# sloisel/MultiGridBarrier.jl

Measured on NVIDIA B200. Metric: mgb_solve DOF*Newton-steps/s (fem2d_P1 ~1.6M DOF, p=1.5), higher is better.
Workload: dtype f64

## Files before the change

multigridbarrier.jl_b200/build.py:

```python
from __future__ import annotations

import os
import shutil
import subprocess
import sys
from concurrent.futures import ThreadPoolExecutor

HERE = os.path.dirname(os.path.abspath(__file__))
CSRC = os.path.join(HERE, "csrc")
OBJ = os.path.join(HERE, "build")
LIB = os.path.join(HERE, "libmgbx.so")
HDR = os.path.join("..", "..", "include", "mgbx.h")
ENGINE = ["engine.hpp", "host_sparse.hpp", "device_common.cuh", "elem_schur.cuh", "node_barrier.cuh", "pcg2.hpp", HDR]
SOURCES = {
    "mgbx.cu": ["mgbx.cu", "host_amg.hpp"] + ENGINE,
    "setup.cu": ["setup.cu", "setup_kernels.cuh"] + ENGINE,
    "evaluate.cu": ["evaluate.cu", "kernels.cuh", "dense_kernels.cuh"] + ENGINE,
    "linear_solve.cu": ["linear_solve.cu", "solver_kernels.cuh"] + ENGINE,
    "newton.cu": ["newton.cu"] + ENGINE,
    "pcg2.cu": ["pcg2.cu", "pcg2.hpp"],
}
FLAGS = ["-gencode", "arch=compute_100a,code=sm_100a", "-O3", "-DNDEBUG", "-lineinfo", "-std=c++17",
         "-Xcompiler", "-fPIC,-O2,-Wall,-Wno-unused-function"]


def nvcc_path():
    for c in (os.environ.get("NVCC"), shutil.which("nvcc"), "/usr/local/cuda/bin/nvcc"):
        if c and os.path.exists(c):
            return c
    raise RuntimeError("nvcc not found")


def _obj(src):
    return os.path.join(OBJ, os.path.splitext(src)[0] + ".o")


def _stale(src):
    o = _obj(src)
    if not os.path.exists(o):
        return True
    t = os.path.getmtime(o)
    return any(os.path.getmtime(os.path.join(CSRC, d)) > t for d in SOURCES[src])

# ... 37 lines not shown
```

multigridbarrier.jl_b200/csrc/device_common.cuh:

```cuda
#pragma once
#include <cuda_runtime.h>
#include <stdint.h>

#include "elem_schur.cuh"
#include "node_barrier.cuh"

namespace mgbx {

#define MGBX_MAX_OPS 8
constexpr int kRedBlocks = 592;
constexpr int kRedThreads = 256;

struct DevCsr {
  int64_t rows = 0, cols = 0, nnz = 0;
  int64_t *ptr = nullptr;
  int32_t *idx = nullptr;
  double *val = nullptr;
};

__device__ __forceinline__ double warp_sum(double v) {
#pragma unroll
  for (int o = 16; o > 0; o >>= 1) v += __shfl_down_sync(0xffffffffu, v, o);
  return v;
}
// ... 245 lines not shown
      "mbarrier.try_wait.parity.shared::cta.b64 p, [%0], %1;\n"
      "@p bra DONE_%=;\n"
      "bra WAIT_%=;\n"
      "DONE_%=:\n"
      "}\n" ::"r"(a),
      "r"(parity)
      : "memory");
}
__device__ __forceinline__ void bulk_g2s(void *smem, const void *gmem, unsigned int bytes, unsigned long long *bar) {
  asm volatile("cp.async.bulk.shared::cluster.global.mbarrier::complete_tx::bytes [%0], [%1], %2, [%3];" ::"r"((unsigned int)__cvta_generic_to_shared(smem)),
               "l"(gmem), "r"(bytes), "r"((unsigned int)__cvta_generic_to_shared(bar))
               : "memory");
}
__device__ __forceinline__ void fence_proxy_async_smem() { asm volatile("fence.proxy.async.shared::cta;" ::: "memory"); }

struct SellPlan {
  int64_t nout = 0, nslices = 0, nterms = 0;
  int64_t *sptr = nullptr;
  int32_t *cnt = nullptr;
  int32_t *src = nullptr;
  double *w = nullptr;
};

__device__ __forceinline__ int64_t csr_find(const DevCsr &A, int64_t row, int32_t col) {
  int64_t lo = A.ptr[row], hi = A.ptr[row + 1];
  while (lo < hi) {
    const int64_t mid = (lo + hi) >> 1;
    const int32_t c = A.idx[mid];
    if (c < col) lo = mid + 1;
    else if (c > col) hi = mid;
    else return mid;
  }
  return -1;
}

constexpr int kCoarseMaxDense = 128;
inline size_t coarse_inverse_smem(int m) { return sizeof(double) * ((size_t)m * (m + 1) + (size_t)m * (m + 1) / 2 + m); }
inline size_t dense_solve_small_smem(int m) { return sizeof(double) * ((size_t)m * (m + 1) + 2 * (size_t)m); }

constexpr int kGemmBM = 64, kGemmBN = 64, kGemmBK = 16, kGemmLd = kGemmBK + 4;

__device__ __forceinline__ void dmma_m8n8k4(double &d0, double &d1, double a, double b) {
  asm volatile("mma.sync.aligned.m8n8k4.row.col.f64.f64.f64.f64 {%0,%1}, {%2}, {%3}, {%0,%1};" : "+d"(d0), "+d"(d1) : "d"(a), "d"(b));
}

constexpr int kCholNB = 64;
// ... 28 lines not shown
```

multigridbarrier.jl_b200/csrc/engine.hpp:

```cpp
#pragma once
#include <cuda_runtime.h>

#include <chrono>
#include <cmath>
#include <cstdio>
#include <cstring>
#include <functional>
#include <map>
#include <memory>
#include <string>
#include <vector>

#include "host_sparse.hpp"
#include "device_common.cuh"
#include "pcg2.hpp"

namespace mgbx {

#define CK(call)                                                                                      \
  do {                                                                                                \
    cudaError_t e_ = (call);                                                                          \
    if (e_ != cudaSuccess)                                                                            \
      throw std::runtime_error(std::string("CUDA error: ") + cudaGetErrorString(e_) + " at " + __FILE__ + ":" + \
                               std::to_string(__LINE__));                                             \
// ... 210 lines not shown
constexpr int kScalPcgOut = 8;
constexpr int kScalTrialSeg = 38;
constexpr int kScalEvalDist = 40;
constexpr int kScalDotSeg = 44;
constexpr int kScalDotSeg2 = 50;
constexpr int kScalSlots = 64;
static_assert(kScalEval + 4 <= kScalDot && kScalDot + 3 <= kScalTrial && kScalTrial + 1 <= kScalSingle &&
                  kScalSingle <= kScalPcgOut && kScalPcgOut + kPcg2OutCount <= kScalTrialSeg &&
                  kScalTrialSeg + 2 == kScalEvalDist && kScalEvalDist + 4 == kScalDotSeg &&
                  kScalDotSeg + 6 <= kScalDotSeg2 && kScalDotSeg2 + 6 <= kScalSlots,
              "scalar slot regions overlap, break the all-reduced range or exceed dscal");

}

struct mgbx_handle {
  mgbx::Pool pool;
  mgbx::Amg amg[2];
  std::string err;
  mgbx_config cfg;
  cudaStream_t stream = nullptr;
  bool has_feas = false;
  double *partials = nullptr;
  unsigned int *ticket = nullptr;
  double *dscal = nullptr;
  double *hscal = nullptr;
  mgbx_step_result *res = nullptr;
  int64_t launches = 0;
  int64_t kc_launches[mgbx::KC_COUNT] = {0};
  double kc_ms[mgbx::KC_COUNT] = {0};
  std::vector<cudaEvent_t> ev_free;
  struct Pending {
    int kc;
    cudaEvent_t a, b;
  };
  std::vector<Pending> ev_pending;
  cudaEvent_t ev_cur = nullptr;
  int pcg2_grid = 0;
  double dgemm_flops = 0.0;
  mgbx::SolveTol last_tol{};
  int rank = 0, nranks = 1;
  void *comm = nullptr;
  int device = -1;
  std::vector<double> prof_ns;
  std::vector<int64_t> prof_cnt;
  std::vector<unsigned long long> prof_host;
};
// ... 73 lines not shown
  void copy(double *dst, const double *src, int64_t m) {
    if (m) CK(cudaMemcpyAsync(dst, src, sizeof(double) * m, cudaMemcpyDeviceToDevice, s));
  }
  void zero(double *dst, int64_t m) {
    if (m) CK(cudaMemsetAsync(dst, 0, sizeof(double) * m, s));
  }
  unsigned int red_grid(int64_t work) {
    const int64_t b = (work + kRedThreads - 1) / kRedThreads;
    return (unsigned int)std::max<int64_t>(1, std::min<int64_t>(b, kRedBlocks));
  }

  bool dist() const { return h->nranks > 1; }
  void allreduce(double *buf, int64_t count, int op = kNcclSum) {
    if (count > 0) NCK(nccl_api().AllReduce(buf, buf, (size_t)count, kNcclFloat64, op, h->comm, s));
  }
  SegList seglist(Amg &A, int J);
  void allreduce_shared(Amg &A, int J, double *v, double *extra = nullptr, int64_t nextra = 0);

  static int group_for(const DevCsr &A) {
    const double avg = A.rows ? (double)A.nnz / (double)A.rows : 0.0;
    return avg > 48.0 ? 32 : (avg > 6.0 ? 4 : 1);
  }
  void spmv(const DevCsr &A, const double *x, const double *y0, double alpha, double *y, int G = 0);
  void axpby(int64_t m, double a, const double *x, double b, const double *y, double *out);
  void prolong_to_fine(Amg &A, int J, const double *x, const double *zbase, double *zf);
  void restrict_from_fine(Amg &A, int J, const double *gb, double *gJ);
  Dot2 dot2(Amg &A, int J, const double *a, const double *b);
  MaxAbs maxabs(int64_t n, const double *v);
  TrialOut eval_trial(Amg &A, int J, double t, double sigma);
  void phase1_slack(Amg &A, Amg &F);
  void blockgrad(Amg &A, const ElemParams &E);
  NodeParams node_params(Amg &A, double t);
  ElemParams elem_params(Amg &A);
  bool elem_fused_setup(Amg &A, const NodeParams &NP, int nex, ElemFused &Q, size_t &smem, unsigned int &grid);
  int plap_dim(const Amg &A) const;
  bool plap_setup(Amg &A, int dim, double t, bool use_bw, PlapParams &Q, size_t &smem, unsigned int &grid, bool cond = true);
  EvalOut eval_f01(Amg &A, int J, double t, const double *zbase, const double *x, double *gout, bool use_bw = true,
                   double *step2 = nullptr);

  System &system_for(Amg &A, int J);
  void assemble(Amg &A, System &S, int J, double t, const double *zbase, const double *x);
  void assemble_unfused(Amg &A, System &S, int J, double t, const double *x);
  void galerkin(System &S, int kend);
  void schur_masks(const Amg &A, const System &S, unsigned &pieces, unsigned &elim) const;
  void assemble_dense(Amg &A, System &S, const NodeParams &P);
  void dgemm_nt(int M, int N, int K, const double *Am, int64_t lda, const double *Bm, int64_t ldb, const double *sc, double *C, int64_t ldc, bool acc, double alpha = 1.0);

  bool precond_fp32(const System &S) const;
  int lambda_power_its(const System &S) const;
  bool use_direct(const System &S, const SysLevel &Lv) const;
  std::vector<int> active_levels(const System &S, int ktop) const;
  void setup_hierarchy(Amg &A, System &S, int ktop);
  void dense_factor(SysLevel &Lv);
  void dense_apply(SysLevel &Lv, const double *b, double *x);
  void direct_solve(SysLevel &Lv, const double *b, double *x);
  SellBuild make_sell(const DevCsr &A, int64_t nthreads);
  void sell_prepare(System &S, int ktop);
  System::Pcg2Dev &pcg2_plan(System &S, int ktop);
  void pcg2_setup_dist(System::Pcg2Dev &D, int nshard);
  SolveResult pcg(System &S, int ktop, const double *b, double *x, const SolveTol &tol);
  SolveResult solve_compact(System &S, int ktop, const double *b, double *x, const SolveTol &tol);
  SolveResult solve(Amg &A, System &S, int J, const double *g, double *dir, const SolveTol &tol);

  struct NewtonOut {
    bool converged;
    int k;
    int status;
    double y, gnorm, inc;
  };
  NewtonOut newton(Amg &A, int J, double t, int maxit, int stop_kind, double lambda_tol, double theta, const mgbx_step_opts &o);
  int step(int which, double t, const mgbx_step_opts &o, mgbx_step_result *r);
  int matched_t(double t_default, double *t_out, double *tstar_out);
};

void solve_kernels_init();
void kron_w_init(size_t smem);

inline bool dense_mode(const Amg &A) { return A.N == 1 && A.p > 64; }

template <class F>
// ... 40 lines not shown
```

multigridbarrier.jl_b200/csrc/evaluate.cu:

```cuda
#include "engine.hpp"
#include "kernels.cuh"
#include "dense_kernels.cuh"

namespace mgbx {
namespace {

template <int MODE>
void launch_node(const NodeParams &P, unsigned int grid, cudaStream_t s) {
  if (P.nD <= 4) k_node<MODE, 4><<<grid, kRedThreads, 0, s>>>(P);
  else if (P.nD <= 6) k_node<MODE, 6><<<grid, kRedThreads, 0, s>>>(P);
  else if (P.nD <= 8) k_node<MODE, 8><<<grid, kRedThreads, 0, s>>>(P);
  else k_node<MODE, MGBX_MAX_ND><<<grid, kRedThreads, 0, s>>>(P);
}

template <auto K, class Params>
void launch_wave(const Params &Q, unsigned int grid, size_t smem, cudaStream_t s) {
  static int nsm[64] = {0};
  int dev = 0;
  CK(cudaGetDevice(&dev));
  if (!nsm[dev]) {
    CK(cudaFuncSetAttribute(K, cudaFuncAttributeMaxDynamicSharedMemorySize, 220 * 1024));
    CK(cudaDeviceGetAttribute(&nsm[dev], cudaDevAttrMultiProcessorCount, dev));
  }
  int occ = 1;
// ... 26 lines not shown
Dot2 dot2_slots(const double *d) { return {d[0], d[1], d[2]}; }
Dot2 dot2_seg_slots(const double *local, const double *shared) {
  return {local[0] + shared[0], local[1] + shared[1], local[2] + shared[2]};
}

}

void kron_w_init(size_t smem) { CK(cudaFuncSetAttribute(k_kron_w, cudaFuncAttributeMaxDynamicSharedMemorySize, (int)smem)); }

void Engine::spmv(const DevCsr &A, const double *x, const double *y0, double alpha, double *y, int G) {
  if (A.rows == 0) return;
  if (G == 0) G = group_for(A);
  pre_launch(KC_SPMV);
  if (G == 32) k_spmv<32><<<nblk(A.rows * 32), 256, 0, s>>>(A, x, y0, alpha, y);
  else if (G == 4) k_spmv<4><<<nblk(A.rows * 4), 256, 0, s>>>(A, x, y0, alpha, y);
  else k_spmv<1><<<nblk(A.rows), 256, 0, s>>>(A, x, y0, alpha, y);
  post_launch(KC_SPMV);
}

void Engine::axpby(int64_t m, double a, const double *x, double b, const double *y, double *out) {
  LAUNCH(KC_VEC, k_axpby<<<nblk(m), 256, 0, s>>>(m, a, x, b, y, out));
}

void Engine::prolong_to_fine(Amg &A, int J, const double *x, const double *zbase, double *zf) {
  const double *v = x;
  for (int l = J; l < A.L - 1; ++l) {
    spmv(A.T[l], v, nullptr, 1.0, A.chain[l + 1]);
    v = A.chain[l + 1];
  }
  spmv(A.RL, v, zbase, 1.0, zf);
}
void Engine::restrict_from_fine(Amg &A, int J, const double *gb, double *gJ) {
  if (J == A.L - 1) {
    spmv(A.RLt, gb, nullptr, 1.0, gJ);
    return;
  }
  spmv(A.RLt, gb, nullptr, 1.0, A.chain2[A.L - 1]);
  const double *v = A.chain2[A.L - 1];
  for (int l = A.L - 2; l >= J; --l) {
    double *out = (l == J) ? gJ : A.chain2[l];
    spmv(A.Tt[l], v, nullptr, 1.0, out);
    v = out;
  }
}


SegList Engine::seglist(Amg &A, int J) {
  SegList S;
  memset(&S, 0, sizeof(S));
  if (J == A.L - 1) {
    S.n = A.nu;
    for (int v = 0; v < A.nu; ++v) {
      S.off[v] = A.voff[J][v];
      S.local[v] = A.var_local[v];
    }
    S.off[A.nu] = A.voff[J][A.nu];
  } else {
    S.n = 1;
    S.off[0] = 0;
    S.off[1] = A.m[J];
  }
  return S;
}
void Engine::allreduce_shared(Amg &A, int J, double *v, double *extra, int64_t nextra) {
  const SegList S = seglist(A, J);
  NCK(nccl_api().GroupStart());
  for (int q = 0; q < S.n; ++q)
    if (!S.local[q]) allreduce(v + S.off[q], S.off[q + 1] - S.off[q]);
// ... 299 lines not shown
    LAUNCH(KC_ELEMG_F2, launch_elem<NODE_F2>(Q, grid, smem, s));
  } else {
    LAUNCH(KC_NODE_F2, launch_node<NODE_F2>(P, red_grid(A.n), s));
    ElemParams E = elem_params(A);
    E.nK = S.nK;
    for (int j = 0; j < S.nK; ++j) E.Krow[j] = S.Krow[j];
    LAUNCH(KC_BLOCKHESS, k_blockhess<<<nblk(S.hblk_size), 256, 0, s>>>(E, S.pl, A.Hn, S.Hblk));
  }
  if (S.elem_local) {
    ElemParams E = elem_params(A);
    E.nK = S.nK;
    for (int j = 0; j < S.nK; ++j) E.Krow[j] = S.Krow[j];
    LAUNCH(KC_COND, k_elem_local_schur<<<nblk(A.N, 128), 128, 0, s>>>(E, S.pl, S.el, A.hEEinv, A.hKE, S.Hblk));
  }
  SysLevel &top = S.lev[0];
  LAUNCH(KC_GATHER, k_sell_gather<<<nblk(top.A.nnz), 256, 0, s>>>(S.top, S.Hblk, top.A.val));
  if (dist()) allreduce(top.A.val, top.A.nnz);
  const int ktop = S.ltop - J;
  setup_hierarchy(A, S, ktop);
  stage_end(STAGE_F2, st);
  if (h->res) h->res->f2_evals++;
}

void Engine::galerkin(System &S, int kend) {
  for (int k = 0; k < kend; ++k) {
    SysLevel &Lv = S.lev[k];
    SysLevel &Lc = S.lev[k + 1];
    if (Lv.T_identity) continue;
    LAUNCH(KC_SPGEMM, k_sell_gather<<<nblk(Lv.AT.nnz), 256, 0, s>>>(Lv.s1, Lv.A.val, Lv.AT.val));
    LAUNCH(KC_SPGEMM, k_sell_gather<<<nblk(Lc.A.nnz), 256, 0, s>>>(Lv.s2, Lv.AT.val, Lc.A.val));
  }
}

void Engine::assemble_unfused(Amg &A, System &S, int J, double t, const double *x) {
  prolong_to_fine(A, J, x, A.z, A.zf);
  NodeParams P = node_params(A, t);
  P.nK = S.nK;
  P.nE = 0;
  for (int j = 0; j < MGBX_MAX_ND; ++j) {
    P.Krow[j] = S.Krow[j];
    P.Erow[j] = -1;
  }
  P.Hn = A.Hn;
  LAUNCH(KC_NODE_F2, launch_node<NODE_F2>(P, red_grid(A.n), s));
  LAUNCH(KC_BLOCKHESS, k_blockhess<<<nblk(S.hblk_size), 256, 0, s>>>(elem_params(A), S.pl, A.Hn, S.Hblk));
  LAUNCH(KC_GATHER, k_sell_gather<<<nblk(S.lev[0].A.nnz), 256, 0, s>>>(S.top, S.Hblk, S.lev[0].A.val));
  if (dist()) allreduce(S.lev[0].A.val, S.lev[0].A.nnz);
  galerkin(S, S.ltop - J);
}


void Engine::dgemm_nt(int M, int N, int K, const double *Am, int64_t lda, const double *Bm, int64_t ldb, const double *sc, double *C, int64_t ldc,
                      bool acc, double alpha) {
  if (M <= 0 || N <= 0) return;
// ... 67 lines not shown
```

multigridbarrier.jl_b200/csrc/kernels.cuh:

```cuda
#pragma once
#include <cuda_runtime.h>
#include <stdint.h>


#include "device_common.cuh"

namespace mgbx {

template <int G>
__global__ void __launch_bounds__(256) k_spmv(DevCsr A, const double *__restrict__ x, const double *y0, double alpha,
                                               double *y) {
  const int64_t gtid = (int64_t)blockIdx.x * blockDim.x + threadIdx.x;
  const int64_t row = gtid / G;
  const int sub = (int)(gtid % G);
  if (row >= A.rows) return;
  const int64_t b = A.ptr[row], e = A.ptr[row + 1];
  double acc = 0.0;
  for (int64_t k = b + sub; k < e; k += G) acc += A.val[k] * x[A.idx[k]];
  if (G > 1) {
#pragma unroll
    for (int o = G / 2; o > 0; o >>= 1) acc += __shfl_down_sync(0xffffffffu, acc, o, G);
  }
  if (sub == 0) y[row] = alpha * acc + (y0 ? y0[row] : 0.0);
}

template <int MODE, int NDT>
__global__ void __launch_bounds__(kRedThreads) k_node(NodeParams P) {
  double red[4] = {0.0, 0.0, 0.0, -INFINITY};
  const int op[4] = {0, 0, 0, 1};
  for (int64_t i = (int64_t)blockIdx.x * blockDim.x + threadIdx.x; i < P.n; i += (int64_t)gridDim.x * blockDim.x) {
    double y[NDT];
    node_Dz(P, i, y);
    if (MODE == NODE_SLACK) {
      const double s = node_slack(P.cd, P.n, i, y);
      P.slack[i] = s;
      red[3] = fmax(red[3], s);
      continue;
    }
    const int nD = P.nD;
    const double bwi = P.bw ? P.bw[i] : 1.0;
    const bool active = !(P.bw && bwi == 0.0);
    double F1[NDT];
    if (MODE == NODE_F01) {
      double F0 = 0.0;
      if (active) F0 = node_eval(P.cd, P.n, i, y, 1, F1, nullptr);
      else
// ... 664 lines not shown
    for (int i = 0; i < p; ++i) {
      const double q = hKE[node0 + i + (int64_t)a * E.n];
      if (q == 0.0) continue;
      if (o < 0) X[i * m + col0 + i] += q;
      else {
        const double *blk = E.ops[o] + e * (int64_t)pp + i;
        for (int c = 0; c < p; ++c) X[i * m + col0 + c] += q * blk[(int64_t)c * p];
      }
    }
  }
  elem_condense(p, nc, Pe, hinv, X, m, EL.R + e * elem_rsize(nc));
  for (int pr = 0; pr < PL.npairs; ++pr) {
    const int ca = (PL.va[pr] == vars[0]) ? 0 : p, cb = (PL.vb[pr] == vars[0]) ? 0 : p;
    double *out = Hblk + ((int64_t)pr * E.N + e) * pp;
    for (int r = 0; r < p; ++r)
      for (int c = 0; c < p; ++c) {
        double s = 0.0;
        for (int i = 0; i < p; ++i) s += X[i * m + ca + r] * X[i * m + cb + c];
        out[r * p + c] += s;
      }
  }
}

__global__ void __launch_bounds__(256) k_sell_gather(SellPlan P, const double *__restrict__ in, double *__restrict__ out) {
  const int64_t nz = (int64_t)blockIdx.x * blockDim.x + threadIdx.x;
  if (nz >= P.nout) return;
  const int64_t off = P.sptr[nz >> 5] + (nz & 31);
  const int c = P.cnt[nz];
  double acc = 0.0;
  if (P.w) {
    for (int k = 0; k < c; ++k) acc += P.w[off + 32 * (int64_t)k] * in[P.src[off + 32 * (int64_t)k]];
  } else {
    for (int k = 0; k < c; ++k) acc += in[P.src[off + 32 * (int64_t)k]];
  }
  out[nz] = acc;
}

}
```

multigridbarrier.jl_b200/csrc/linear_solve.cu:

```cuda
#include "engine.hpp"
#include "solver_kernels.cuh"

namespace mgbx {

void solve_kernels_init() {
  CK(cudaFuncSetAttribute(k_coarse_inverse, cudaFuncAttributeMaxDynamicSharedMemorySize, (int)coarse_inverse_smem(kCoarseMaxDense)));
  CK(cudaFuncSetAttribute(k_dense_solve_small, cudaFuncAttributeMaxDynamicSharedMemorySize, (int)dense_solve_small_smem(kCoarseMaxDense)));
  CK(cudaFuncSetAttribute(k_chol_diag_inv, cudaFuncAttributeMaxDynamicSharedMemorySize, (int)kCholDiagSmem));
  CK(cudaFuncSetAttribute(k_chol_solve_blocked, cudaFuncAttributeMaxDynamicSharedMemorySize, (int)(sizeof(double) * kDenseMaxUnknowns)));
}

bool Engine::precond_fp32(const System &S) const {
  if (h->cfg.precond_fp32 != 2) return h->cfg.precond_fp32 == 1;
  int64_t tot = 0;
  for (const SysLevel &Lv : S.lev) tot += Lv.A.nnz;
  return tot >= 10000000;
}
int Engine::lambda_power_its(const System &S) const {
  if (h->cfg.lambda_power >= 0) return h->cfg.lambda_power;
  if (S.lev.empty() || S.lev[0].A.rows == 0) return 0;
  return ((double)S.lev[0].A.nnz / (double)S.lev[0].A.rows > 16.0) ? 6 : 0;
}
bool Engine::use_direct(const System &S, const SysLevel &Lv) const {
  return S.dense || Lv.m <= h->cfg.dense_direct_max;
}
std::vector<int> Engine::active_levels(const System &S, int ktop) const {
  const int nlev = (int)S.lev.size();
  const int kend = (S.cut >= 0) ? std::max(S.cut, ktop) : nlev - 1;
  std::vector<int> act;
  for (int k = ktop; k <= kend; ++k) {
    if (k < kend && S.lev[k].T_identity) continue;
    act.push_back(k);
  }
  return act;
}

void Engine::setup_hierarchy(Amg &A, System &S, int ktop) {
  const int nlev = (int)S.lev.size();
  SysLevel &Ltop = S.lev[ktop];
  const bool direct = use_direct(S, Ltop);
  int kend = ktop;
  if (!direct) kend = (S.cut >= 0) ? std::max(S.cut, ktop) : nlev - 1;
  galerkin(S, kend);
  if (direct) {
    if (Ltop.m > kCoarseMaxDense) dense_factor(Ltop);
    return;
  }
  for (int k = ktop; k <= kend; ++k) {
    SysLevel &Lv = S.lev[k];
    CK(cudaMemsetAsync(Lv.lam, 0, sizeof(double), s));
    LAUNCH(KC_VEC, k_l1diag<<<nblk(Lv.m), 256, 0, s>>>(Lv.A, Lv.dinv, Lv.diag, (unsigned long long *)Lv.lam));
    if (precond_fp32(S)) {
      if (!Lv.val32) Lv.val32 = h->pool.alloc<float>(Lv.A.nnz);
      LAUNCH(KC_VEC, k_f64_to_f32<<<nblk(Lv.A.nnz), 256, 0, s>>>(Lv.A.nnz, Lv.A.val, Lv.val32));
    }
  }
  if (S.cut >= 0 && S.cut >= ktop) {
    SysLevel &Lc = S.lev[S.cut];
    const int m = (int)Lc.m;
    if (!Lc.dense_inv) Lc.dense_inv = h->pool.alloc<double>((size_t)m * m);
    LAUNCH(KC_DENSE, k_coarse_inverse<<<1, 1024, coarse_inverse_smem(m), s>>>(Lc.A, Lc.dense_inv));
  }
  sell_prepare(S, ktop);
  if (lambda_power_its(S) > 0) {
    System::Pcg2Dev &D = pcg2_plan(S, ktop);
    if ((int64_t)D.host.nlev * h->pcg2_grid > 3 * (int64_t)kPcg2MaxGrid) throw std::runtime_error("internal: too many levels for the power-iteration kernel");
    LAUNCH(KC_VEC, CK(pcg2_lambda_power(D.dev, h->pcg2_grid, lambda_power_its(S), 1.2, s)));
  }
}

void Engine::dense_factor(SysLevel &Lv) {
  const int m = (int)Lv.m;
  if (m == 0) return;
  const int npan = (m + kCholNB - 1) / kCholNB;
  if (!Lv.dense) {
    Lv.dense = h->pool.alloc<double>((size_t)m * m);
    Lv.dscale = h->pool.alloc<double>(m);
    Lv.dense_inv = h->pool.alloc<double>((size_t)npan * kCholNB * kCholNB);
  }
  zero(Lv.dense, (int64_t)m * m);
  LAUNCH(KC_DENSE, k_dense_scale_diag<<<nblk(m), 256, 0, s>>>(Lv.A, Lv.dscale));
  LAUNCH(KC_DENSE, k_csr_to_dense<<<nblk(m), 256, 0, s>>>(Lv.A, Lv.dscale, Lv.dense));
  for (int p = 0; p < npan; ++p) {
    const int k0 = p * kCholNB, nb = std::min(kCholNB, m - k0), rem = m - k0 - nb;
    double *Li = Lv.dense_inv + (size_t)p * kCholNB * kCholNB;
    LAUNCH(KC_DENSE, k_chol_diag_inv<<<1, 1024, kCholDiagSmem, s>>>(Lv.dense, m, k0, Li));
// ... 45 lines not shown
  std::vector<int> soff(nsl + 1, 0);
  int64_t tot = 0;
  for (int q = 0; q < nsl; ++q) {
    tot += 32 * (int64_t)hw[q];
    if (tot > INT32_MAX) throw std::runtime_error("persistent solve kernel: sliced-ELL level matrix exceeds 32-bit indexing");
    soff[q + 1] = (int)tot;
  }
  B.M.entries = (int)tot;
  B.soff = h->pool.upload<int>(soff.data(), soff.size(), s);
  B.idx = h->pool.alloc<int>((size_t)tot);
  B.src = h->pool.alloc<int>((size_t)tot);
  B.val = h->pool.alloc<double>((size_t)tot);
  B.valf = h->pool.alloc<float>((size_t)tot);
  CK(sell_fill_pattern(A.rows, lpr, A.ptr, A.idx, B.soff, B.idx, B.src, s));
  h->launches += 2;
  B.M.soff = B.soff;
  B.M.idx = B.idx;
  B.M.val = B.val;
  B.M.valf = nullptr;
  CK(cudaStreamSynchronize(s));
  return B;
}

void Engine::sell_prepare(System &S, int ktop) {
  const std::vector<int> act = active_levels(S, ktop);
  const int64_t grid_threads = (int64_t)h->pcg2_grid * kPcg2Threads;
  for (size_t q = 0; q < act.size(); ++q) {
    SysLevel &Lv = S.lev[act[q]];
    const int64_t nthr = (q > 0 && Lv.m <= h->cfg.tail_max) ? kPcg2Threads : grid_threads;
    if (!Lv.sell_A) {
      Lv.sA = make_sell(Lv.A, nthr);
      Lv.sell_A = true;
    }
    if (Lv.sA.M.entries) LAUNCH(KC_VEC, CK(sell_fill_values(Lv.sA.M.entries, Lv.sA.src, Lv.A.val, Lv.sA.val, Lv.sA.valf, s)));
    if (q + 1 < act.size() && !Lv.sell_T) {
      const int64_t nthr_c = (S.lev[act[q + 1]].m <= h->cfg.tail_max) ? kPcg2Threads : grid_threads;
      Lv.sT = make_sell(Lv.T, nthr);
      Lv.sTt = make_sell(Lv.Tt, nthr_c);
      if (Lv.sT.M.entries) LAUNCH(KC_VEC, CK(sell_fill_values(Lv.sT.M.entries, Lv.sT.src, Lv.T.val, Lv.sT.val, Lv.sT.valf, s)));
      if (Lv.sTt.M.entries) LAUNCH(KC_VEC, CK(sell_fill_values(Lv.sTt.M.entries, Lv.sTt.src, Lv.Tt.val, Lv.sTt.val, Lv.sTt.valf, s)));
      Lv.sell_T = true;
    }
  }
}

System::Pcg2Dev &Engine::pcg2_plan(System &S, int ktop) {
  auto it = S.pplans2.find(ktop);
  if (it != S.pplans2.end()) return it->second;
  System::Pcg2Dev &D = S.pplans2[ktop];
  Pcg2Plan &P = D.host;
  P = Pcg2Plan();
  const std::vector<int> act = active_levels(S, ktop);
  if ((int)act.size() > kPcg2MaxLevels) throw std::runtime_error("persistent solve kernel: too many levels");
  P.nlev = (int)act.size();
  P.bottom_dense = (S.cut >= 0 && act.back() == S.cut) ? 1 : 0;
  P.nu = std::max(1, h->cfg.smoother_sweeps);
  P.nu_bottom = 30;
// ... 259 lines not shown
```

multigridbarrier.jl_b200/csrc/mgbx.cu:

```cuda
#include <dlfcn.h>

#include <numeric>

#include "engine.hpp"
#include "host_amg.hpp"

using namespace mgbx;

namespace {

thread_local std::string g_last_error;
const char *kKClassNames[KC_COUNT] = {"node_f01", "node_f2", "blockgrad", "blockhess", "csr_gather", "spmv", "spgemm",
                                             "vector", "condense", "dense", "pcg_persistent", "elem_f01", "elem_f2", "dgemm_dmma", "elem_generic_f01", "elem_generic_f2"};

Amg &amg_arg(mgbx_handle *h, int which, const char *prefix = "") {
  if (which < 0 || which > 1 || (which == 1 && !h->has_feas)) throw ArgError(std::string(prefix) + "no such AMG");
  return h->amg[which];
}
Amg &level_arg(mgbx_handle *h, int which, int level) {
  Amg &A = amg_arg(h, which);
  if (level < 0 || level >= A.L) throw ArgError("no such level");
  return A;
}

// ... 131 lines not shown
    if (h->cfg.persistent != 2) throw ArgError("mgbx_config.persistent must be 2 (the only solve kernel)");
    int ndev = 0;
    cudaError_t e = cudaGetDeviceCount(&ndev);
    if (e != cudaSuccess || ndev == 0)
      throw std::runtime_error("CUDA device required: libmgbx has no CPU fallback (cudaGetDeviceCount: " +
                               std::string(cudaGetErrorString(e)) + ")");
    if (h->cfg.device >= 0) CK(cudaSetDevice(h->cfg.device));
    CK(cudaGetDevice(&h->device));
    CK(cudaStreamCreateWithFlags(&h->stream, cudaStreamNonBlocking));
    h->pool.stream = h->stream;
    {
      int dev = 0;
      CK(cudaGetDevice(&dev));
      cudaMemPool_t mp = nullptr;
      CK(cudaDeviceGetDefaultMemPool(&mp, dev));
      uint64_t keep = UINT64_MAX;
      CK(cudaMemPoolSetAttribute(mp, cudaMemPoolAttrReleaseThreshold, &keep));
      h->pcg2_grid = pcg2_grid(dev);
      if (h->pcg2_grid == 0) throw std::runtime_error("CUDA device cannot run the cooperative solve kernel");
      solve_kernels_init();
    }
    h->partials = h->pool.zeros<double>((size_t)kRedBlocks * 8, h->stream);
    h->ticket = h->pool.zeros<unsigned int>(4, h->stream);
    h->dscal = h->pool.zeros<double>(kScalSlots, h->stream);
    CK(cudaMallocHost((void **)&h->hscal, sizeof(double) * kScalSlots));
    const mgbx_amg &a0 = prob->amg[0];
    create_amg(h, a0, h->amg[0]);
    Amg &A = h->amg[0];
    if (!prob->f_grid || !prob->g_grid) throw ArgError("f_grid / g_grid missing");
    CK(cudaMemcpyAsync(A.f, prob->f_grid, sizeof(double) * A.n * A.nD, cudaMemcpyHostToDevice, h->stream));
    CK(cudaMemcpyAsync(A.z, prob->g_grid, sizeof(double) * A.n * A.nu, cudaMemcpyHostToDevice, h->stream));
    CK(cudaMemcpyAsync(A.zinit, prob->g_grid, sizeof(double) * A.n * A.nu, cudaMemcpyHostToDevice, h->stream));
    if (prob->barrier_weights) A.bw = h->pool.upload<double>(prob->barrier_weights, A.n, h->stream);
    HostTimer tq;
    upload_convex(h, prob->Q, A.n, A.nD, A.cd);
    if (h->cfg.verbose > 0) fprintf(stderr, "[mgbx] convex set scanned + uploaded %.3fs\n", tq.lap());
    if (prob->amg[1].n > 0) attach_feasibility(h, prob->amg[1]);
    CK(cudaStreamSynchronize(h->stream));
    return MGBX_OK;
  });
  if (rc != MGBX_OK) {
    g_last_error = h->err;
    mgbx_destroy(h);
    return rc;
  }
  *out = h;
// ... 495 lines not shown
```

multigridbarrier.jl_b200/csrc/pcg2.cu:

```cuda
#include "pcg2.hpp"

#include <math.h>

namespace mgbx {
namespace {

__device__ __forceinline__ double warp_sum2(double v) {
#pragma unroll
  for (int o = 16; o > 0; o >>= 1) v += __shfl_down_sync(0xffffffffu, v, o);
  return v;
}

__device__ __forceinline__ void grid_barrier2(unsigned int *bar) {
  __syncthreads();
  if (threadIdx.x == 0) {
    unsigned int nb = 1;
    if (blockIdx.x == 0) nb = 0x80000000u - (gridDim.x - 1);
    unsigned int old, cur;
    asm volatile("atom.add.release.gpu.u32 %0,[%1],%2;" : "=r"(old) : "l"(bar), "r"(nb) : "memory");
    int spins = 0;
    do {
      asm volatile("ld.acquire.gpu.u32 %0,[%1];" : "=r"(cur) : "l"(bar) : "memory");
      if (++spins > 64) __nanosleep(40);
    } while (((old ^ cur) & 0x80000000u) == 0);
  }
  __syncthreads();
}

enum { PK_FIRST2 = 0, PK_PRE = 1, PK_RESID = 2, PK_RESTRICT = 3, PK_TAIL = 4, PK_PROLONG = 5, PK_POST = 6, PK_DENSE = 7, PK_RZSUM = 8, PK_MATVEC = 9,
       PK_UPDATE = 10, PK_INIT = 11 };
__device__ __forceinline__ void prof_mark(unsigned long long *prof, int tag) {
  if (prof && blockIdx.x == 0 && threadIdx.x == 0) {
    unsigned long long t;
    asm volatile("mov.u64 %0, %%globaltimer;" : "=l"(t));
    const unsigned long long n = prof[0];
    if (n + 1 < (unsigned long long)kPcg2ProfCap) {
      prof[1 + 2 * n] = (unsigned long long)tag;
      prof[2 + 2 * n] = t;
      prof[0] = n + 1;
    }
  }
}

template <bool GRID>
struct Ld {
  static __device__ __forceinline__ int i(const int *p) { return GRID ? __ldg(p) : *p; }
  static __device__ __forceinline__ double m(const double *p) { return GRID ? __ldg(p) : *p; }
  static __device__ __forceinline__ float mf(const float *p) { return GRID ? __ldg(p) : *p; }
  static __device__ __forceinline__ double v(const double *p) { return GRID ? __ldcg(p) : *p; }
// ... 749 lines not shown
  const int64_t nsl = (rows + rps - 1) / rps;
  if (gw >= nsl) return;
  const int64_t row = gw * rps + lane / lpr;
  const int b = soff[gw], w = (soff[gw + 1] - b) / 32;
  const int64_t p0 = row < rows ? ptr[row] : 0;
  const int len = row < rows ? (int)(ptr[row + 1] - p0) : 0;
  const int pad = len > 0 ? cidx[p0] : 0;
  for (int j = 0; j < w; ++j) {
    const int e = b + 32 * j + lane;
    const int k = j * lpr + sub;
    if (k < len) {
      idx[e] = cidx[p0 + k];
      src[e] = (int)(p0 + k);
    } else {
      idx[e] = pad;
      src[e] = -1;
    }
  }
}

__global__ void k_sell_values(int entries, const int *__restrict__ src, const double *__restrict__ cval, double *val, float *valf) {
  const int e = blockIdx.x * blockDim.x + threadIdx.x;
  if (e >= entries) return;
  const int q = src[e];
  const double v = q >= 0 ? cval[q] : 0.0;
  val[e] = v;
  if (valf) valf[e] = (float)v;
}

}

size_t pcg2_tail_bytes(const Pcg2Plan &P) {
  auto al = [](size_t b) { return (b + 15) & ~(size_t)15; };
  auto sell = [&](const SellMat &M) -> size_t {
    if (M.nslices == 0) return 0;
    return al(sizeof(int) * (M.nslices + 1)) + al(sizeof(int) * (size_t)M.entries) + al(sizeof(float) * (size_t)M.entries);
  };
  size_t tot = 0;
  for (int k = P.nbig; k < P.nlev; ++k) {
    const Pcg2Level &L = P.lev[k];
    const bool dense_bottom = (k == P.nlev - 1) && P.bottom_dense;
    tot += (dense_bottom ? 0 : sell(L.A)) + sell(L.T) + sell(L.Tt) + 6 * al(sizeof(double) * (size_t)L.m);
  }
  return tot;
}

static int g_pcg2_grid[64] = {0};

int pcg2_grid(int device) {
  if (device < 0 || device >= 64) return 0;
// ... 61 lines not shown
```

multigridbarrier.jl_b200/csrc/solver_kernels.cuh:

```cuda
#pragma once

#include "device_common.cuh"

namespace mgbx {

__global__ void __launch_bounds__(256) k_condense_rhs(CondParams P, const double *__restrict__ g, double *Gt) {
  const int64_t i = (int64_t)blockIdx.x * blockDim.x + threadIdx.x;
  if (i >= P.n) return;
  double gE[4], tE[4], Hi[16];
  const int nE = P.nE;
  for (int ev = 0; ev < nE; ++ev) gE[ev] = g[P.Eoff[ev] + i];
  int q = 0;
  for (int a = 0; a < nE; ++a)
    for (int b = a; b < nE; ++b, ++q) {
      const double v = P.hEEinv[i + (int64_t)q * P.n];
      Hi[a * nE + b] = v;
      Hi[b * nE + a] = v;
    }
  for (int ev = 0; ev < nE; ++ev) {
    double s = 0.0;
    for (int ew = 0; ew < nE; ++ew) s += Hi[ev * nE + ew] * gE[ew];
    tE[ev] = s;
  }
  for (int a = 0; a < P.nK; ++a) {
// ... 51 lines not shown
  const int nc = EL.nc, p = NP.p;
  double rc[kElemMaxNc];
  const int64_t col = P.Eoff[0] + EL.c0[e];
  for (int k = 0; k < nc; ++k) rc[k] = g[col + k];
  for (int r = 0; r < p; ++r) {
    const int64_t i = e * p + r;
    double y[MGBX_MAX_ND];
    node_Dz(NP, i, y);
    double s = 0.0;
    for (int a = 0; a < P.nK; ++a) s += P.hKE[i + (int64_t)a * P.n] * y[P.Krow[a]];
    for (int k = 0; k < nc; ++k) rc[k] -= EL.P[i * nc + k] * s;
  }
  elem_hss_solve(nc, EL.R + e * elem_rsize(nc), rc);
  for (int k = 0; k < nc; ++k) x[col + k] = rc[k];
}

__global__ void k_pw_init(int64_t m, double *v) {
  const int64_t i = (int64_t)blockIdx.x * blockDim.x + threadIdx.x;
  if (i < m) v[i] = 1.0 + 0.5 * cos(0.7 * (double)i) + ((i & 1) ? 0.25 : -0.25);
}

__global__ void __launch_bounds__(256) k_l1diag(DevCsr A, double *dinv, double *diag, unsigned long long *lam_bits) {
  const int64_t row = (int64_t)blockIdx.x * blockDim.x + threadIdx.x;
  double ratio = 0.0;
  if (row < A.rows) {
    double s = 0.0, d = 0.0;
    for (int64_t k = A.ptr[row]; k < A.ptr[row + 1]; ++k) {
      s += fabs(A.val[k]);
      if (A.idx[k] == row) d = A.val[k];
    }
    dinv[row] = s > 0.0 ? 1.0 / s : 0.0;
    if (diag) diag[row] = d > 0.0 ? 1.0 / d : 0.0;
    if (d > 0.0 && isfinite(s)) ratio = s / d;
  }
  if (lam_bits) {
    ratio = warp_max(ratio);
    if ((threadIdx.x & 31) == 0 && ratio > 0.0) atomicMax(lam_bits, (unsigned long long)__double_as_longlong(ratio));
  }
}

__global__ void k_dense_scale_diag(DevCsr A, double *d) {
  const int64_t row = (int64_t)blockIdx.x * blockDim.x + threadIdx.x;
  if (row >= A.rows) return;
  double dg = 0.0;
  for (int64_t k = A.ptr[row]; k < A.ptr[row + 1]; ++k)
    if (A.idx[k] == row) dg = A.val[k];
  d[row] = dg > 0.0 ? 1.0 / sqrt(dg) : 1.0;
}

__global__ void k_csr_to_dense(DevCsr A, const double *d, double *Ad) {
  const int64_t row = (int64_t)blockIdx.x * blockDim.x + threadIdx.x;
  if (row >= A.rows) return;
  const double di = d[row];
  for (int64_t k = A.ptr[row]; k < A.ptr[row + 1]; ++k) Ad[row * A.rows + A.idx[k]] = A.val[k] * di * d[A.idx[k]];
}

__global__ void __launch_bounds__(256) k_dense_symv(const double *__restrict__ M, int m, const double *__restrict__ x, double *y) {
// ... 293 lines not shown
```

Before: 504.3 million.

## Batch small multigrid SpMV, gather and setup kernels into one cooperative walk kernel

Adds a persistent cooperative kernel, k_walk, that runs a list of small steps inside one launch, separated by software grid barriers. The steps are SpMV, SELL gathers, l1-diagonal computation and SELL value fills. Prolongation and restriction chains, Galerkin products and the preconditioner setup on small coarse levels now go through it instead of one launch per level. Steps above a size threshold still get their own ordinary launch. The aim is to cut kernel-launch and tail overhead on coarse levels, at the cost of grid-barrier synchronisation and a large parameter struct per launch.

```diff
diff --git a/multigridbarrier.jl_b200/build.py b/multigridbarrier.jl_b200/build.py
--- a/multigridbarrier.jl_b200/build.py
+++ b/multigridbarrier.jl_b200/build.py
@@ -18,7 +18,7 @@
     "evaluate.cu": ["evaluate.cu", "kernels.cuh", "dense_kernels.cuh"] + ENGINE,
     "linear_solve.cu": ["linear_solve.cu", "solver_kernels.cuh"] + ENGINE,
     "newton.cu": ["newton.cu"] + ENGINE,
-    "pcg2.cu": ["pcg2.cu", "pcg2.hpp"],
+    "pcg2.cu": ["pcg2.cu", "pcg2.hpp", "device_common.cuh", "elem_schur.cuh", "node_barrier.cuh"],
 }
 FLAGS = ["-gencode", "arch=compute_100a,code=sm_100a", "-O3", "-DNDEBUG", "-lineinfo", "-std=c++17",
          "-Xcompiler", "-fPIC,-O2,-Wall,-Wno-unused-function"]
diff --git a/multigridbarrier.jl_b200/csrc/device_common.cuh b/multigridbarrier.jl_b200/csrc/device_common.cuh
--- a/multigridbarrier.jl_b200/csrc/device_common.cuh
+++ b/multigridbarrier.jl_b200/csrc/device_common.cuh
@@ -291,6 +291,64 @@
   double *w = nullptr;
 };
 
+__device__ __forceinline__ void grid_barrier2(unsigned int *bar) {
+  __syncthreads();
+  if (threadIdx.x == 0) {
+    unsigned int nb = 1;
+    if (blockIdx.x == 0) nb = 0x80000000u - (gridDim.x - 1);
+    unsigned int old, cur;
+    asm volatile("atom.add.release.gpu.u32 %0,[%1],%2;" : "=r"(old) : "l"(bar), "r"(nb) : "memory");
+    int spins = 0;
+    do {
+      asm volatile("ld.acquire.gpu.u32 %0,[%1];" : "=r"(cur) : "l"(bar) : "memory");
+      if (++spins > 64) __nanosleep(40);
+    } while (((old ^ cur) & 0x80000000u) == 0);
+  }
+  __syncthreads();
+}
+
+enum WalkOp { WALK_SPMV = 0, WALK_GATHER = 1, WALK_L1DIAG = 2, WALK_SELLVAL = 3 };
+struct WalkStep {
+  int op, same_phase;
+  int G;
+  DevCsr A;
+  SellPlan P;
+  const double *x, *y0;
+  double alpha;
+  double *y, *y2;
+  unsigned long long *bits;
+  const int *src;
+  float *yf;
+  int64_t n;
+};
+constexpr int kWalkMaxSteps = 20;
+constexpr int kWalkThreads = 1024;
+struct WalkSteps {
+  int n;
+  WalkStep st[kWalkMaxSteps];
+};
+
+__device__ __forceinline__ double l1diag_row(const DevCsr &A, double *dinv, double *diag, int64_t row) {
+  double ratio = 0.0;
+  if (row < A.rows) {
+    double s = 0.0, d = 0.0;
+    for (int64_t k = A.ptr[row]; k < A.ptr[row + 1]; ++k) {
+      s += fabs(A.val[k]);
+      if (A.idx[k] == row) d = A.val[k];
+    }
+    dinv[row] = s > 0.0 ? 1.0 / s : 0.0;
+    if (diag) diag[row] = d > 0.0 ? 1.0 / d : 0.0;
+    if (d > 0.0 && isfinite(s)) ratio = s / d;
+  }
+  return ratio;
+}
+__device__ __forceinline__ void sell_value_entry(const int *src, const double *cval, double *val, float *valf, int64_t e) {
+  const int q = src[e];
+  const double v = q >= 0 ? cval[q] : 0.0;
+  val[e] = v;
+  if (valf) valf[e] = (float)v;
+}
+
 __device__ __forceinline__ int64_t csr_find(const DevCsr &A, int64_t row, int32_t col) {
   int64_t lo = A.ptr[row], hi = A.ptr[row + 1];
   while (lo < hi) {
diff --git a/multigridbarrier.jl_b200/csrc/engine.hpp b/multigridbarrier.jl_b200/csrc/engine.hpp
--- a/multigridbarrier.jl_b200/csrc/engine.hpp
+++ b/multigridbarrier.jl_b200/csrc/engine.hpp
@@ -256,6 +256,7 @@
   bool has_feas = false;
   double *partials = nullptr;
   unsigned int *ticket = nullptr;
+  unsigned int *walk_bar = nullptr;
   double *dscal = nullptr;
   double *hscal = nullptr;
   mgbx_step_result *res = nullptr;
@@ -375,6 +376,10 @@
     return avg > 48.0 ? 32 : (avg > 6.0 ? 4 : 1);
   }
   void spmv(const DevCsr &A, const double *x, const double *y0, double alpha, double *y, int G = 0);
+  static WalkStep spmv_step(const DevCsr &A, const double *x, const double *y0, double alpha, double *y);
+  static WalkStep gather_step(const SellPlan &P, const double *x, double *y);
+  void walk(const std::vector<WalkStep> &steps, int kc);
+  static constexpr int64_t kWalkOwnLaunch = 2000 * 256;
   void axpby(int64_t m, double a, const double *x, double b, const double *y, double *out);
   void prolong_to_fine(Amg &A, int J, const double *x, const double *zbase, double *zf);
   void restrict_from_fine(Amg &A, int J, const double *gb, double *gJ);
@@ -395,6 +400,7 @@
   void assemble(Amg &A, System &S, int J, double t, const double *zbase, const double *x);
   void assemble_unfused(Amg &A, System &S, int J, double t, const double *x);
   void galerkin(System &S, int kend);
+  void galerkin_steps(System &S, int kend, std::vector<WalkStep> &steps);
   void schur_masks(const Amg &A, const System &S, unsigned &pieces, unsigned &elim) const;
   void assemble_dense(Amg &A, System &S, const NodeParams &P);
   void dgemm_nt(int M, int N, int K, const double *Am, int64_t lda, const double *Bm, int64_t ldb, const double *sc, double *C, int64_t ldc, bool acc, double alpha = 1.0);
@@ -408,7 +414,7 @@
   void dense_apply(SysLevel &Lv, const double *b, double *x);
   void direct_solve(SysLevel &Lv, const double *b, double *x);
   SellBuild make_sell(const DevCsr &A, int64_t nthreads);
-  void sell_prepare(System &S, int ktop);
+  void sell_prepare(System &S, int ktop, std::vector<WalkStep> &steps);
   System::Pcg2Dev &pcg2_plan(System &S, int ktop);
   void pcg2_setup_dist(System::Pcg2Dev &D, int nshard);
   SolveResult pcg(System &S, int ktop, const double *b, double *x, const SolveTol &tol);
diff --git a/multigridbarrier.jl_b200/csrc/evaluate.cu b/multigridbarrier.jl_b200/csrc/evaluate.cu
--- a/multigridbarrier.jl_b200/csrc/evaluate.cu
+++ b/multigridbarrier.jl_b200/csrc/evaluate.cu
@@ -72,28 +72,75 @@
   LAUNCH(KC_VEC, k_axpby<<<nblk(m), 256, 0, s>>>(m, a, x, b, y, out));
 }
 
+WalkStep Engine::spmv_step(const DevCsr &A, const double *x, const double *y0, double alpha, double *y) {
+  WalkStep w{};
+  w.op = WALK_SPMV;
+  w.G = group_for(A);
+  w.A = A;
+  w.x = x;
+  w.y0 = y0;
+  w.alpha = alpha;
+  w.y = y;
+  return w;
+}
+WalkStep Engine::gather_step(const SellPlan &P, const double *x, double *y) {
+  WalkStep w{};
+  w.op = WALK_GATHER;
+  w.P = P;
+  w.x = x;
+  w.y = y;
+  return w;
+}
+
+void Engine::walk(const std::vector<WalkStep> &steps, int kc) {
+  WalkSteps W;
+  W.n = 0;
+  auto flush = [&]() {
+    const WalkStep &w = W.st[0];
+    if (W.n == 1 && w.op == WALK_SPMV) spmv(w.A, w.x, w.y0, w.alpha, w.y, w.G);
+    else if (W.n == 1 && w.op == WALK_GATHER) LAUNCH(kc, k_sell_gather<<<nblk(w.P.nout), 256, 0, s>>>(w.P, w.x, w.y));
+    else if (W.n > 0) {
+      unsigned int *bar = h->walk_bar;
+      void *args[] = {(void *)&W, (void *)&bar};
+      LAUNCH(kc, CK(cudaLaunchCooperativeKernel((const void *)k_walk, dim3(h->pcg2_grid), dim3(kWalkThreads), args, 0, s)));
+    }
+    W.n = 0;
+  };
+  for (const WalkStep &w : steps) {
+    const int64_t work = w.op == WALK_SPMV ? w.A.rows * w.G : w.op == WALK_GATHER ? w.P.nout : w.op == WALK_L1DIAG ? w.A.rows : w.n;
+    if (work == 0) continue;
+    if ((w.op == WALK_SPMV || w.op == WALK_GATHER) && work >= kWalkOwnLaunch) {
+      flush();
+      W.st[W.n++] = w;
+      flush();
+      continue;
+    }
+    if (W.n == kWalkMaxSteps) flush();
+    W.st[W.n++] = w;
+  }
+  flush();
+}
+
 void Engine::prolong_to_fine(Amg &A, int J, const double *x, const double *zbase, double *zf) {
+  std::vector<WalkStep> st;
   const double *v = x;
   for (int l = J; l < A.L - 1; ++l) {
-    spmv(A.T[l], v, nullptr, 1.0, A.chain[l + 1]);
+    st.push_back(spmv_step(A.T[l], v, nullptr, 1.0, A.chain[l + 1]));
     v = A.chain[l + 1];
   }
-  spmv(A.RL, v, zbase, 1.0, zf);
+  st.push_back(spmv_step(A.RL, v, zbase, 1.0, zf));
+  walk(st, KC_SPMV);
 }
 void Engine::restrict_from_fine(Amg &A, int J, const double *gb, double *gJ) {
-  if (J == A.L - 1) {
-    spmv(A.RLt, gb, nullptr, 1.0, gJ);
-    return;
-  }
-  spmv(A.RLt, gb, nullptr, 1.0, A.chain2[A.L - 1]);
-  const double *v = A.chain2[A.L - 1];
-  for (int l = A.L - 2; l >= J; --l) {
+  std::vector<WalkStep> st;
+  const double *v = gb;
+  for (int l = A.L - 1; l >= J; --l) {
     double *out = (l == J) ? gJ : A.chain2[l];
-    spmv(A.Tt[l], v, nullptr, 1.0, out);
+    st.push_back(spmv_step(l == A.L - 1 ? A.RLt : A.Tt[l], v, nullptr, 1.0, out));
     v = out;
   }
-}
-
+  walk(st, KC_SPMV);
+}
 
 SegList Engine::seglist(Amg &A, int J) {
   SegList S;
@@ -439,14 +486,19 @@
   if (h->res) h->res->f2_evals++;
 }
 
-void Engine::galerkin(System &S, int kend) {
+void Engine::galerkin_steps(System &S, int kend, std::vector<WalkStep> &steps) {
   for (int k = 0; k < kend; ++k) {
     SysLevel &Lv = S.lev[k];
     SysLevel &Lc = S.lev[k + 1];
     if (Lv.T_identity) continue;
-    LAUNCH(KC_SPGEMM, k_sell_gather<<<nblk(Lv.AT.nnz), 256, 0, s>>>(Lv.s1, Lv.A.val, Lv.AT.val));
-    LAUNCH(KC_SPGEMM, k_sell_gather<<<nblk(Lc.A.nnz), 256, 0, s>>>(Lv.s2, Lv.AT.val, Lc.A.val));
-  }
+    steps.push_back(gather_step(Lv.s1, Lv.A.val, Lv.AT.val));
+    steps.push_back(gather_step(Lv.s2, Lv.AT.val, Lc.A.val));
+  }
+}
+void Engine::galerkin(System &S, int kend) {
+  std::vector<WalkStep> st;
+  galerkin_steps(S, kend, st);
+  walk(st, KC_SPGEMM);
 }
 
 void Engine::assemble_unfused(Amg &A, System &S, int J, double t, const double *x) {
diff --git a/multigridbarrier.jl_b200/csrc/kernels.cuh b/multigridbarrier.jl_b200/csrc/kernels.cuh
--- a/multigridbarrier.jl_b200/csrc/kernels.cuh
+++ b/multigridbarrier.jl_b200/csrc/kernels.cuh
@@ -6,22 +6,28 @@
 #include "device_common.cuh"
 
 namespace mgbx {
+
+template <int G>
+__device__ __forceinline__ void spmv_row(const DevCsr &A, const double *x, const double *y0, double alpha, double *y, int64_t gtid) {
+  const int64_t row = gtid / G;
+  const int sub = (int)(gtid % G);
+  const bool in = row < A.rows;
+  const int64_t b = in ? A.ptr[row] : 0, e = in ? A.ptr[row + 1] : 0;
+  double acc = 0.0;
+  for (int64_t k = b + sub; k < e; k += G) acc += A.val[k] * x[A.idx[k]];
+  if (G > 1) {
+#pragma unroll
+    for (int o = G / 2; o > 0; o >>= 1) acc += __shfl_down_sync(0xffffffffu, acc, o, G);
+  }
+  if (in && sub == 0) y[row] = alpha * acc + (y0 ? y0[row] : 0.0);
+}
 
 template <int G>
 __global__ void __launch_bounds__(256) k_spmv(DevCsr A, const double *__restrict__ x, const double *y0, double alpha,
                                                double *y) {
   const int64_t gtid = (int64_t)blockIdx.x * blockDim.x + threadIdx.x;
-  const int64_t row = gtid / G;
-  const int sub = (int)(gtid % G);
-  if (row >= A.rows) return;
-  const int64_t b = A.ptr[row], e = A.ptr[row + 1];
-  double acc = 0.0;
-  for (int64_t k = b + sub; k < e; k += G) acc += A.val[k] * x[A.idx[k]];
-  if (G > 1) {
-#pragma unroll
-    for (int o = G / 2; o > 0; o >>= 1) acc += __shfl_down_sync(0xffffffffu, acc, o, G);
-  }
-  if (sub == 0) y[row] = alpha * acc + (y0 ? y0[row] : 0.0);
+  if (gtid / G >= A.rows) return;
+  spmv_row<G>(A, x, y0, alpha, y, gtid);
 }
 
 template <int MODE, int NDT>
@@ -732,9 +738,7 @@
   }
 }
 
-__global__ void __launch_bounds__(256) k_sell_gather(SellPlan P, const double *__restrict__ in, double *__restrict__ out) {
-  const int64_t nz = (int64_t)blockIdx.x * blockDim.x + threadIdx.x;
-  if (nz >= P.nout) return;
+__device__ __forceinline__ void sell_gather_entry(const SellPlan &P, const double *in, double *out, int64_t nz) {
   const int64_t off = P.sptr[nz >> 5] + (nz & 31);
   const int c = P.cnt[nz];
   double acc = 0.0;
@@ -746,4 +750,36 @@
   out[nz] = acc;
 }
 
-}
+__global__ void __launch_bounds__(256) k_sell_gather(SellPlan P, const double *__restrict__ in, double *__restrict__ out) {
+  const int64_t nz = (int64_t)blockIdx.x * blockDim.x + threadIdx.x;
+  if (nz >= P.nout) return;
+  sell_gather_entry(P, in, out, nz);
+}
+
+__global__ void __launch_bounds__(kWalkThreads, 1) k_walk(WalkSteps W, unsigned int *bar) {
+  const int64_t first = (int64_t)blockIdx.x * blockDim.x, stride = (int64_t)gridDim.x * blockDim.x;
+  for (int i = 0; i < W.n; ++i) {
+    const WalkStep &S = W.st[i];
+    if (i && !S.same_phase) grid_barrier2(bar);
+    if (S.op == WALK_GATHER) {
+      for (int64_t nz = first + threadIdx.x; nz < S.P.nout; nz += stride) sell_gather_entry(S.P, S.x, S.y, nz);
+    } else if (S.op == WALK_SELLVAL) {
+      for (int64_t e = first + threadIdx.x; e < S.n; e += stride) sell_value_entry(S.src, S.x, S.y, S.yf, e);
+    } else if (S.op == WALK_L1DIAG) {
+      for (int64_t b = first; b < S.A.rows; b += stride) {
+        double ratio = warp_max(l1diag_row(S.A, S.y, S.y2, b + threadIdx.x));
+        if ((threadIdx.x & 31) == 0 && ratio > 0.0) atomicMax(S.bits, (unsigned long long)__double_as_longlong(ratio));
+      }
+    } else {
+      const int64_t work = S.A.rows * S.G;
+      for (int64_t b = first; b < work; b += stride) {
+        const int64_t gtid = b + threadIdx.x;
+        if (S.G == 32) spmv_row<32>(S.A, S.x, S.y0, S.alpha, S.y, gtid);
+        else if (S.G == 4) spmv_row<4>(S.A, S.x, S.y0, S.alpha, S.y, gtid);
+        else spmv_row<1>(S.A, S.x, S.y0, S.alpha, S.y, gtid);
+      }
+    }
+  }
+}
+
+}
diff --git a/multigridbarrier.jl_b200/csrc/linear_solve.cu b/multigridbarrier.jl_b200/csrc/linear_solve.cu
--- a/multigridbarrier.jl_b200/csrc/linear_solve.cu
+++ b/multigridbarrier.jl_b200/csrc/linear_solve.cu
@@ -41,15 +41,38 @@
   const bool direct = use_direct(S, Ltop);
   int kend = ktop;
   if (!direct) kend = (S.cut >= 0) ? std::max(S.cut, ktop) : nlev - 1;
-  galerkin(S, kend);
+  std::vector<WalkStep> steps;
+  galerkin_steps(S, kend, steps);
+  const size_t nprod = steps.size();
   if (direct) {
+    walk(steps, KC_SPGEMM);
     if (Ltop.m > kCoarseMaxDense) dense_factor(Ltop);
     return;
   }
   for (int k = ktop; k <= kend; ++k) {
     SysLevel &Lv = S.lev[k];
     CK(cudaMemsetAsync(Lv.lam, 0, sizeof(double), s));
-    LAUNCH(KC_VEC, k_l1diag<<<nblk(Lv.m), 256, 0, s>>>(Lv.A, Lv.dinv, Lv.diag, (unsigned long long *)Lv.lam));
+    if (Lv.m >= kWalkOwnLaunch) continue;
+    WalkStep w{};
+    w.op = WALK_L1DIAG;
+    w.same_phase = 1;
+    w.A = Lv.A;
+    w.y = Lv.dinv;
+    w.y2 = Lv.diag;
+    w.bits = (unsigned long long *)Lv.lam;
+    steps.push_back(w);
+  }
+  sell_prepare(S, ktop, steps);
+  if (steps.size() > nprod) steps[nprod].same_phase = 0;
+  walk(steps, KC_SPGEMM);
+  for (int k : active_levels(S, ktop)) {
+    SysLevel &Lv = S.lev[k];
+    if (Lv.sA.M.entries >= kWalkOwnLaunch) LAUNCH(KC_VEC, CK(sell_fill_values(Lv.sA.M.entries, Lv.sA.src, Lv.A.val, Lv.sA.val, Lv.sA.valf, s)));
+  }
+  for (int k = ktop; k <= kend; ++k) {
+    SysLevel &Lv = S.lev[k];
+    if (Lv.m >= kWalkOwnLaunch)
+      LAUNCH(KC_VEC, k_l1diag<<<nblk(Lv.m), 256, 0, s>>>(Lv.A, Lv.dinv, Lv.diag, (unsigned long long *)Lv.lam));
     if (precond_fp32(S)) {
       if (!Lv.val32) Lv.val32 = h->pool.alloc<float>(Lv.A.nnz);
       LAUNCH(KC_VEC, k_f64_to_f32<<<nblk(Lv.A.nnz), 256, 0, s>>>(Lv.A.nnz, Lv.A.val, Lv.val32));
@@ -61,7 +84,6 @@
     if (!Lc.dense_inv) Lc.dense_inv = h->pool.alloc<double>((size_t)m * m);
     LAUNCH(KC_DENSE, k_coarse_inverse<<<1, 1024, coarse_inverse_smem(m), s>>>(Lc.A, Lc.dense_inv));
   }
-  sell_prepare(S, ktop);
   if (lambda_power_its(S) > 0) {
     System::Pcg2Dev &D = pcg2_plan(S, ktop);
     if ((int64_t)D.host.nlev * h->pcg2_grid > 3 * (int64_t)kPcg2MaxGrid) throw std::runtime_error("internal: too many levels for the power-iteration kernel");
@@ -153,7 +175,7 @@
   return B;
 }
 
-void Engine::sell_prepare(System &S, int ktop) {
+void Engine::sell_prepare(System &S, int ktop, std::vector<WalkStep> &steps) {
   const std::vector<int> act = active_levels(S, ktop);
   const int64_t grid_threads = (int64_t)h->pcg2_grid * kPcg2Threads;
   for (size_t q = 0; q < act.size(); ++q) {
@@ -163,7 +185,17 @@
       Lv.sA = make_sell(Lv.A, nthr);
       Lv.sell_A = true;
     }
-    if (Lv.sA.M.entries) LAUNCH(KC_VEC, CK(sell_fill_values(Lv.sA.M.entries, Lv.sA.src, Lv.A.val, Lv.sA.val, Lv.sA.valf, s)));
+    if (Lv.sA.M.entries) {
+      WalkStep w{};
+      w.op = WALK_SELLVAL;
+      w.same_phase = 1;
+      w.n = Lv.sA.M.entries;
+      w.src = Lv.sA.src;
+      w.x = Lv.A.val;
+      w.y = Lv.sA.val;
+      w.yf = Lv.sA.valf;
+      if (w.n < kWalkOwnLaunch) steps.push_back(w);
+    }
     if (q + 1 < act.size() && !Lv.sell_T) {
       const int64_t nthr_c = (S.lev[act[q + 1]].m <= h->cfg.tail_max) ? kPcg2Threads : grid_threads;
       Lv.sT = make_sell(Lv.T, nthr);
diff --git a/multigridbarrier.jl_b200/csrc/mgbx.cu b/multigridbarrier.jl_b200/csrc/mgbx.cu
--- a/multigridbarrier.jl_b200/csrc/mgbx.cu
+++ b/multigridbarrier.jl_b200/csrc/mgbx.cu
@@ -177,6 +177,7 @@
     }
     h->partials = h->pool.zeros<double>((size_t)kRedBlocks * 8, h->stream);
     h->ticket = h->pool.zeros<unsigned int>(4, h->stream);
+    h->walk_bar = h->pool.zeros<unsigned int>(1, h->stream);
     h->dscal = h->pool.zeros<double>(kScalSlots, h->stream);
     CK(cudaMallocHost((void **)&h->hscal, sizeof(double) * kScalSlots));
     const mgbx_amg &a0 = prob->amg[0];
diff --git a/multigridbarrier.jl_b200/csrc/pcg2.cu b/multigridbarrier.jl_b200/csrc/pcg2.cu
--- a/multigridbarrier.jl_b200/csrc/pcg2.cu
+++ b/multigridbarrier.jl_b200/csrc/pcg2.cu
@@ -1,4 +1,5 @@
 #include "pcg2.hpp"
+#include "device_common.cuh"
 
 #include <math.h>
 
@@ -9,22 +10,6 @@
 #pragma unroll
   for (int o = 16; o > 0; o >>= 1) v += __shfl_down_sync(0xffffffffu, v, o);
   return v;
-}
-
-__device__ __forceinline__ void grid_barrier2(unsigned int *bar) {
-  __syncthreads();
-  if (threadIdx.x == 0) {
-    unsigned int nb = 1;
-    if (blockIdx.x == 0) nb = 0x80000000u - (gridDim.x - 1);
-    unsigned int old, cur;
-    asm volatile("atom.add.release.gpu.u32 %0,[%1],%2;" : "=r"(old) : "l"(bar), "r"(nb) : "memory");
-    int spins = 0;
-    do {
-      asm volatile("ld.acquire.gpu.u32 %0,[%1];" : "=r"(cur) : "l"(bar) : "memory");
-      if (++spins > 64) __nanosleep(40);
-    } while (((old ^ cur) & 0x80000000u) == 0);
-  }
-  __syncthreads();
 }
 
 enum { PK_FIRST2 = 0, PK_PRE = 1, PK_RESID = 2, PK_RESTRICT = 3, PK_TAIL = 4, PK_PROLONG = 5, PK_POST = 6, PK_DENSE = 7, PK_RZSUM = 8, PK_MATVEC = 9,
@@ -820,10 +805,7 @@
 __global__ void k_sell_values(int entries, const int *__restrict__ src, const double *__restrict__ cval, double *val, float *valf) {
   const int e = blockIdx.x * blockDim.x + threadIdx.x;
   if (e >= entries) return;
-  const int q = src[e];
-  const double v = q >= 0 ? cval[q] : 0.0;
-  val[e] = v;
-  if (valf) valf[e] = (float)v;
+  sell_value_entry(src, cval, val, valf, e);
 }
 
 }
diff --git a/multigridbarrier.jl_b200/csrc/solver_kernels.cuh b/multigridbarrier.jl_b200/csrc/solver_kernels.cuh
--- a/multigridbarrier.jl_b200/csrc/solver_kernels.cuh
+++ b/multigridbarrier.jl_b200/csrc/solver_kernels.cuh
@@ -97,17 +97,7 @@
 
 __global__ void __launch_bounds__(256) k_l1diag(DevCsr A, double *dinv, double *diag, unsigned long long *lam_bits) {
   const int64_t row = (int64_t)blockIdx.x * blockDim.x + threadIdx.x;
-  double ratio = 0.0;
-  if (row < A.rows) {
-    double s = 0.0, d = 0.0;
-    for (int64_t k = A.ptr[row]; k < A.ptr[row + 1]; ++k) {
-      s += fabs(A.val[k]);
-      if (A.idx[k] == row) d = A.val[k];
-    }
-    dinv[row] = s > 0.0 ? 1.0 / s : 0.0;
-    if (diag) diag[row] = d > 0.0 ? 1.0 / d : 0.0;
-    if (d > 0.0 && isfinite(s)) ratio = s / d;
-  }
+  double ratio = l1diag_row(A, dinv, diag, row);
   if (lam_bits) {
     ratio = warp_max(ratio);
     if ((threadIdx.x & 31) == 0 && ratio > 0.0) atomicMax(lam_bits, (unsigned long long)__double_as_longlong(ratio));
```

New measurement: 514.4 million (median of 6 runs). 2.0% higher.
